# huang-yh/SelfOcc

Measured on NVIDIA H100. Metric: rendered rays/sec (6-cam 900x1600), higher is better.
Workload: dtype f32

## Files before the change

### include/selfocc_b200.h

```cpp
#ifndef SELFOCC_B200_H
#define SELFOCC_B200_H

#include <stdint.h>

#ifdef __cplusplus
extern "C" {
#endif

#define SO_OK 0
#define SO_ERR_INVALID_ARG (-1)
#define SO_ERR_UNSUPPORTED (-2)
#define SO_ERR_CUDA (-3)
#define SO_ERR_NO_DEVICE (-4)

#define SO_ABI_VERSION 9

int so_abi_version(void);
int so_last_cuda_error(void);
const char* so_error_string(int code);
int64_t so_launch_count(void);

#define SO_PROF_NUM_TAGS 10
int so_profile_enable(int on);
int so_profile_reset(void);
// ... 107 lines not shown
                          int32_t n_sem, const uint8_t* lut, uint8_t* occ, uint8_t* sem, void* stream);
int so_occ_sample_labels(const float* vol_sdf, const float* vol_feat, const so_volume_desc* vol_host, const float* xs,
                         int32_t nx, const float* ys, int32_t ny, const float* zs, int32_t nz, const float* points, int64_t m,
                         float thresh, int32_t sem_begin, int32_t n_sem, const uint8_t* lut, uint8_t* occ, uint8_t* sem,
                         void* stream);
int so_occ_confusion(const uint8_t* pred, const uint8_t* gt, const uint8_t* mask, int64_t n, int32_t n_cls, int32_t ignore,
                     int64_t* counts, void* stream);

int so_msda_forward(const float* value, const int64_t* spatial_shapes, const int64_t* level_start_index,
                    const float* loc, const float* weights, float* out,
                    int32_t B, int32_t Nv, int32_t Hd, int32_t Dh, int32_t Nq, int32_t L, int32_t P,
                    void* stream);

int so_msda_backward(const float* value, const int64_t* spatial_shapes, const int64_t* level_start_index,
                     const float* loc, const float* weights, const float* grad_out,
                     float* grad_value, float* grad_loc, float* grad_weights,
                     int32_t B, int32_t Nv, int32_t Hd, int32_t Dh, int32_t Nq, int32_t L, int32_t P,
                     void* stream);

int so_linear_force_ss(int on);
int so_split_tf32(const float* w, float* w_hi, float* w_lo, int64_t n, void* stream);
int so_linear_3xtf32(const float* x, const float* w_hi, const float* w_lo, const float* bias, const float* residual,
                     float* y, int64_t M, int32_t N, int32_t K, int32_t relu, void* stream);

int so_linear_3xtf32_ln(const float* x, const float* w_hi, const float* w_lo, const float* bias, const float* residual,
                        const float* gamma, const float* beta, float eps, float* y, int64_t M, int32_t N, int32_t K,
                        int32_t relu, void* stream);

int so_layer_norm(const float* x, const float* add, const float* gamma, const float* beta, float* y, int64_t rows,
                  int32_t C, float eps, void* stream);

int so_flatten_level(const float* feat, const float* cams_embeds, const float* level_embed, float* out, int32_t N, int32_t C,
                     int32_t hw, int64_t level_start, int64_t total, void* stream);

int so_point_sampling(const float* ref_3d, const float* lidar2img, int32_t D, int32_t Q, int32_t N,
                      float img_h, float img_w, float* uv, uint8_t* mask, uint8_t* vis, void* stream);

int so_point_sampling_scaled(const float* ref_3d, const float* lidar2img, const float* scale_xy, int32_t D,
                             int32_t Q, int32_t N, float img_h, float img_w, float* uv, uint8_t* mask,
                             uint8_t* vis, void* stream);

int so_tpv_cross_attn_forward(const float* value, const int64_t* spatial_shapes,
                              const int64_t* level_start_index, const float* offsets, const float* logits,
                              const float* uv, const uint8_t* vis, float* slots, int32_t* count,
                              int32_t N, int32_t Nv, int32_t Hd, int32_t Dh, int32_t Q, int32_t L, int32_t D,
                              void* stream);

int so_tpv_cross_attn_forward_strided(const float* value, const int64_t* spatial_shapes, const int64_t* level_start_index,
                                      const float* offsets, const float* logits, const float* uv, const uint8_t* vis,
                                      float* slots, int32_t* count, int32_t N, int32_t Nv, int32_t Hd, int32_t Dh, int32_t Q,
                                      int32_t L, int32_t D, int32_t value_ld, int32_t offsets_ld, int32_t logits_ld, void* stream);

int so_attn_force_v1(int on);

int so_visible_index_lists(const uint8_t* mask, int32_t N, int32_t Q, int32_t D,
                           int64_t* index_lists, int32_t* lens, void* stream);

int so_tpv_self_attn_forward(const float* value, const int64_t* spatial_shapes,
                             const int64_t* level_start_index, const float* offsets, const float* logits,
                             const float* ref, float* out,
                             int32_t Nv, int32_t Hd, int32_t Dh, int32_t Q, int32_t L, int32_t P,
                             void* stream);

int so_tpv_self_attn_forward_strided(const float* value, const int64_t* spatial_shapes, const int64_t* level_start_index,
                                     const float* offsets, const float* logits, const float* ref, float* out, int32_t Nv,
                                     int32_t Hd, int32_t Dh, int32_t Q, int32_t L, int32_t P, int32_t value_ld,
                                     int32_t offsets_ld, int32_t logits_ld, void* stream);

int so_tpv_cross_attn_backward(const float* value, const int64_t* spatial_shapes, const int64_t* level_start_index,
                               const float* offsets, const float* logits, const float* uv, const uint8_t* vis,
                               const int32_t* count, const float* grad_slots, float* grad_value, float* grad_offsets,
                               float* grad_logits, int32_t N, int32_t Nv, int32_t Hd, int32_t Dh, int32_t Q, int32_t L,
                               int32_t D, void* stream);

int so_tpv_self_attn_backward(const float* value, const int64_t* spatial_shapes, const int64_t* level_start_index,
                              const float* offsets, const float* logits, const float* ref, const float* grad_out,
                              float* grad_value, float* grad_offsets, float* grad_logits, int32_t Nv, int32_t Hd, int32_t Dh,
                              int32_t Q, int32_t L, int32_t P, void* stream);

#define SO_REPROJ_COMBINE 0
#define SO_REPROJ_MULTI_NEW 1
int so_reproj_stats_forward(const float* weights, const float* ts, const float* deltas, const float* pix,
                            const float* img2prev, const float* img2next, const float* curr_imgs, const float* prev_imgs,
                            const float* next_imgs, int32_t n_cam, int32_t rays_per_cam, int32_t S, int32_t img_h,
                            int32_t img_w, float size_h, float size_w, int32_t mode, float* stats, float* colours,
                            void* stream);
int so_reproj_stats_backward(const float* ts, const float* deltas, const float* pix, const float* img2prev,
                             const float* img2next, const float* curr_imgs, const float* prev_imgs, const float* next_imgs,
                             int32_t n_cam, int32_t rays_per_cam, int32_t S, int32_t img_h, int32_t img_w, float size_h,
                             float size_w, int32_t mode, const float* stats, const float* grad_stats, float* grad_weights,
                             void* stream);

#define SO_SAMPLE_MEAN_EIKONAL 0
#define SO_SAMPLE_MEAN_ABS 1
#define SO_SAMPLE_MEAN_NEG_RELU 2
#define SO_SAMPLE_MEAN_WORKSPACE_BYTES 8192
int so_sample_mean_forward(const float* x, int64_t n, int32_t op, void* workspace, float* out, void* stream);
int so_sample_mean_backward(const float* x, int64_t n, int32_t op, const float* grad_out, float* grad_x, void* stream);

#ifdef __cplusplus
}
#endif
#endif
```

### selfocc_b200/_lib.py

```python
import ctypes as C
import os

_PKG = os.path.dirname(os.path.abspath(__file__))
LIB_PATH = os.environ.get('SELFOCC_B200_LIB') or os.path.join(_PKG, 'lib', 'libselfocc_b200.so')
ABI_VERSION = 9


class AxisMap(C.Structure):
    _fields_ = [('start', C.c_float), ('range0', C.c_float), ('range1', C.c_float), ('size0', C.c_float),
                ('size1', C.c_float), ('offset', C.c_float)]


class VolumeDesc(C.Structure):
    _fields_ = [('H', C.c_int32), ('W', C.c_int32), ('Z', C.c_int32), ('zpitch', C.c_int32),
                ('n_feat', C.c_int32), ('feat_pitch', C.c_int32), ('axis', AxisMap * 3)]


class RayDesc(C.Structure):
    _fields_ = [('n_cam', C.c_int32), ('rays_per_cam', C.c_int32), ('nx', C.c_int32), ('ny', C.c_int32),
                ('sx', C.c_float), ('ox', C.c_float), ('sy', C.c_float), ('oy', C.c_float),
                ('ray_begin', C.c_int64), ('ray_count', C.c_int64), ('chunk_len', C.c_int64)]


class RenderParams(C.Structure):
# ... 6 lines not shown
_I = C.c_int32
_L = C.c_int64
_F = C.c_float

SIGNATURES = {
    'so_abi_version': (C.c_int, []),
    'so_last_cuda_error': (C.c_int, []),
    'so_error_string': (C.c_char_p, [C.c_int]),
    'so_launch_count': (C.c_int64, []),
    'so_profile_enable': (C.c_int, [C.c_int]),
    'so_profile_reset': (C.c_int, []),
    'so_profile_elapsed_ms': (C.c_int, [C.c_int, C.POINTER(C.c_float), C.POINTER(C.c_int32)]),
    'so_tpv_decode': (C.c_int, [_P, _P, _P, _I, _P, _P, _P, _P, C.POINTER(VolumeDesc), _P, _P, _P]),
    'so_tpv_decode_rows': (C.c_int, [_P, _P, _P, _I, _P, _P, _P, _P, C.POINTER(VolumeDesc), _I, _I, _P, _P, _P]),
    'so_tpv_decode_bwd_features': (C.c_int, [_P, _P, _P, _I, C.POINTER(VolumeDesc), _I, _I, _P, _P]),
    'so_tpv_decode_bwd_hidden': (C.c_int, [_P, _P, _P, _P, _I, C.POINTER(VolumeDesc), _I, _I, _P, _P, _P]),
    'so_tpv_decode_bwd_input': (C.c_int, [_P, _P, _L, _P]),
    'so_tpv_decode_force_simt': (C.c_int, [C.c_int]),
    'so_render_train_force_fwd32': (C.c_int, [C.c_int]),
    'so_render_train_force_sem_generic': (C.c_int, [C.c_int]),
    'so_render_workspace_floats': (C.c_int64, [_L]),
    'so_render_infer': (C.c_int, [_P, _P, C.POINTER(VolumeDesc), _P, _P, C.POINTER(RayDesc), C.POINTER(RenderParams),
                                  _P, _P, _P, _P, _P, _P, _P, _P, _P, _P]),
    'so_render_pack_floats': (_L, [C.POINTER(VolumeDesc)]),
    'so_render_pack': (C.c_int, [_P, _P, C.POINTER(VolumeDesc), _P, _P]),
    'so_render_infer_packed': (C.c_int, [_P, _P, C.POINTER(VolumeDesc), _P, _P, _P, C.POINTER(RayDesc), C.POINTER(RenderParams),
                                         _P, _P, _P, _P, _P, _P, _P, _P, _P, _P, _P]),
    'so_render_train_forward': (C.c_int, [_P, _P, C.POINTER(VolumeDesc), _P, _P, C.POINTER(RayDesc), C.POINTER(RenderParams),
                                          _P, _P] + [_P] * 11 + [_P, _P, _P]),
    'so_render_train_pair_floats': (_L, [C.POINTER(VolumeDesc)]),
    'so_render_train_backward': (C.c_int, [_P, _P, C.POINTER(VolumeDesc), _P, _P, C.POINTER(RayDesc), C.POINTER(RenderParams),
                                           _P, _P] + [_P] * 7 + [_P, _P, _P, _P, _P]),
    'so_render_train_probe': (C.c_int, [C.POINTER(VolumeDesc), _P, _P, C.POINTER(RayDesc), C.POINTER(RenderParams), _P, _P, _P]),
    'so_field_query_backward': (C.c_int, [C.POINTER(VolumeDesc), _P, _L, _P, _P, _P, _P, _P, _P]),
    'so_field_second_grad': (C.c_int, [_P, C.POINTER(VolumeDesc), _P, _L, _P, _P]),
    'so_field_second_grad_backward': (C.c_int, [C.POINTER(VolumeDesc), _P, _L, _P, _P, _P]),
    'so_depth_metric_sample': (C.c_int, [_P, _P, _I, _I, _I, _I, _P, _P]),
    'so_depth_metric_sums': (C.c_int, [_P, _P, _P, _P, _I, _I, _P, _P]),
    'so_field_query': (C.c_int, [_P, _P, C.POINTER(VolumeDesc), _P, _L, _P, _P, _P, _P]),
    'so_msda_forward': (C.c_int, [_P, _P, _P, _P, _P, _P, _I, _I, _I, _I, _I, _I, _I, _P]),
    'so_msda_backward': (C.c_int, [_P, _P, _P, _P, _P, _P, _P, _P, _P, _I, _I, _I, _I, _I, _I, _I, _P]),
    'so_linear_force_ss': (C.c_int, [C.c_int]),
    'so_split_tf32': (C.c_int, [_P, _P, _P, _L, _P]),
    'so_linear_3xtf32': (C.c_int, [_P, _P, _P, _P, _P, _P, _L, _I, _I, _I, _P]),
    'so_linear_3xtf32_ln': (C.c_int, [_P, _P, _P, _P, _P, _P, _P, _F, _P, _L, _I, _I, _I, _P]),
    'so_flatten_level': (C.c_int, [_P, _P, _P, _P, _I, _I, _I, _L, _L, _P]),
    'so_layer_norm': (C.c_int, [_P, _P, _P, _P, _P, _L, _I, _F, _P]),
    'so_point_sampling': (C.c_int, [_P, _P, _I, _I, _I, _F, _F, _P, _P, _P, _P]),
    'so_point_sampling_scaled': (C.c_int, [_P, _P, _P, _I, _I, _I, _F, _F, _P, _P, _P, _P]),
    'so_tpv_cross_attn_forward': (C.c_int, [_P, _P, _P, _P, _P, _P, _P, _P, _P, _I, _I, _I, _I, _I, _I, _I, _P]),
    'so_tpv_cross_attn_forward_strided': (C.c_int, [_P, _P, _P, _P, _P, _P, _P, _P, _P] + [_I] * 10 + [_P]),
    'so_tpv_self_attn_forward_strided': (C.c_int, [_P, _P, _P, _P, _P, _P, _P] + [_I] * 9 + [_P]),
    'so_attn_force_v1': (C.c_int, [C.c_int]),
    'so_visible_index_lists': (C.c_int, [_P, _I, _I, _I, _P, _P, _P]),
    'so_tpv_self_attn_forward': (C.c_int, [_P, _P, _P, _P, _P, _P, _P, _I, _I, _I, _I, _I, _I, _P]),
    'so_tpv_cross_attn_backward': (C.c_int, [_P] * 12 + [_I] * 7 + [_P]),
    'so_tpv_self_attn_backward': (C.c_int, [_P] * 10 + [_I] * 6 + [_P]),
    'so_reproj_stats_forward': (C.c_int, [_P] * 9 + [_I] * 5 + [_F, _F, _I, _P, _P, _P]),
    'so_reproj_stats_backward': (C.c_int, [_P] * 8 + [_I] * 5 + [_F, _F, _I, _P, _P, _P, _P]),
    'so_occ_lattice_labels': (C.c_int, [_P, _P, C.POINTER(VolumeDesc), _P, _I, _P, _I, _P, _I, _F, _I, _I, _P, _P, _P, _P]),
    'so_occ_sample_labels': (C.c_int, [_P, _P, C.POINTER(VolumeDesc), _P, _I, _P, _I, _P, _I, _P, _L, _F, _I, _I, _P, _P, _P, _P]),
    'so_occ_confusion': (C.c_int, [_P, _P, _P, _L, _I, _I, _P, _P]),
    'so_sample_mean_forward': (C.c_int, [_P, _L, _I, _P, _P, _P]),
    'so_sample_mean_backward': (C.c_int, [_P, _L, _I, _P, _P, _P]),
}

_lib = None


class SelfOccLibraryError(RuntimeError):
    pass


def load():
    global _lib
    if _lib is not None:
        return _lib
    if not os.path.exists(LIB_PATH):
        raise SelfOccLibraryError(
            'libselfocc_b200.so not found at %s -- run `python -c "import __graft_entry__ as g; g.build()"` '
            '(there is no CPU/PyTorch fallback for the hot path)' % LIB_PATH)
    lib = C.CDLL(LIB_PATH)
    for name, (res, args) in SIGNATURES.items():
        try:
            fn = getattr(lib, name)
        except AttributeError as e:
            raise SelfOccLibraryError('symbol %s missing from %s' % (name, LIB_PATH)) from e
        fn.restype = res
        fn.argtypes = args
    if lib.so_abi_version() != ABI_VERSION:
        raise SelfOccLibraryError('ABI version mismatch: library %d, binding %d' % (lib.so_abi_version(), ABI_VERSION))
    _lib = lib
    return lib


def check(code, what):
    if code != 0:
        lib = load()
        raise SelfOccLibraryError('%s failed: %s (code %d, cudaError %d)' % (
            what, lib.so_error_string(code).decode(), code, lib.so_last_cuda_error()))


def launch_count():
    return int(load().so_launch_count())


# ... 23 lines not shown
```

### selfocc_b200/csrc/gemm.cu

```cuda
#include "tc_common.cuh"

namespace so {

constexpr int kGemmConsumers = 256;
constexpr int kGemmThreads = kGemmConsumers + 32;
constexpr int kGemmTileM = kWgRows;
constexpr int kGemmTileBytes = kGemmTileM * 128;
constexpr int kMaxStages = 12;
constexpr int kMaxBN = 128;

typedef CUresult (*EncodeTiledFn)(CUtensorMap*, CUtensorMapDataType, cuuint32_t, void*, const cuuint64_t*, const cuuint64_t*,
                                  const cuuint32_t*, const cuuint32_t*, CUtensorMapInterleave, CUtensorMapSwizzle,
                                  CUtensorMapL2promotion, CUtensorMapFloatOOBfill);

static EncodeTiledFn get_encode_fn() {
  static EncodeTiledFn fn = nullptr;
  if (!fn) {
    void* p = nullptr;
    cudaDriverEntryPointQueryResult q;
    if (cudaGetDriverEntryPoint("cuTensorMapEncodeTiled", &p, cudaEnableDefault, &q) == cudaSuccess && q == cudaDriverEntryPointSuccess)
      fn = reinterpret_cast<EncodeTiledFn>(p);
  }
  return fn;
}
// ... 38 lines not shown
    const long long c = bn_cost(bn, N, m_tiles, sms, nullptr, nullptr);
    if (c < best_cost) { best = bn; best_cost = c; }
  }
  return best;
}

static PipeCfg make_pipe_cfg(int64_t M, int N, int K, bool reg_a, bool whole_row, int sms) {
  PipeCfg c;
  c.m_tiles = (int)ceil_div64(M, kGemmTileM);
  c.BN = pick_bn(N, c.m_tiles, sms, whole_row);
  bn_cost(c.BN, N, c.m_tiles, sms, &c.n_tiles, &c.groups);
  c.KA = K / kAtomK;
  c.w_bytes = 2 * c.KA * c.BN * 128;
  c.stage_bytes = reg_a ? kGemmTileBytes : 2 * kGemmTileBytes;
  const int fixed = c.w_bytes + 256;
  c.stages = (227 * 1024 - 1024 - fixed) / c.stage_bytes & ~1;
  if (c.stages > kMaxStages) c.stages = kMaxStages;
  c.smem = fixed + c.stages * c.stage_bytes + 1024;
  return c;
}

template <int NR>
__device__ __forceinline__ void fence_regs(float* r) {
#pragma unroll
  for (int i = 0; i < NR; ++i) asm volatile("" : "+f"(r[i])::"memory");
}
template <int NR>
__device__ __forceinline__ void fence_regs(uint32_t* r) {
#pragma unroll
  for (int i = 0; i < NR; ++i) asm volatile("" : "+r"(r[i])::"memory");
}

__device__ __forceinline__ void ring_advance(int& s, uint32_t& ph, int n) {
  if (++s == n) { s = 0; ph ^= 1; }
}

__device__ __forceinline__ void load_split_frag(const uint8_t* stage, int frag_row, int g, int t, uint32_t* ah, uint32_t* al) {
  const uint8_t* r0 = stage + frag_row * 128 + 4 * t;
#pragma unroll
  for (int kk = 0; kk < 4; ++kk) {
    const float v[4] = {*reinterpret_cast<const float*>(r0 + (((2 * kk) ^ g) << 4)),
                        *reinterpret_cast<const float*>(r0 + 8 * 128 + (((2 * kk) ^ g) << 4)),
                        *reinterpret_cast<const float*>(r0 + (((2 * kk + 1) ^ g) << 4)),
                        *reinterpret_cast<const float*>(r0 + 8 * 128 + (((2 * kk + 1) ^ g) << 4))};
#pragma unroll
    for (int i = 0; i < 4; ++i) {
      const float h = tf32_rn(v[i]);
      ah[4 * kk + i] = __float_as_uint(h);
      al[4 * kk + i] = __float_as_uint(v[i] - h);
    }
  }
  fence_regs<16>(ah);
  fence_regs<16>(al);
}

template <int BN>
__device__ __forceinline__ void mma_atom_rs(float* acc, uint32_t* ah, uint32_t* al, uint32_t bhi, uint32_t blo, uint32_t& accum) {
  fence_regs<BN / 2>(acc);
  wg_fence();
#pragma unroll
  for (int prod = 0; prod < 3; ++prod) {
    const uint32_t* af = prod == 1 ? al : ah;
    const uint32_t bb = prod == 2 ? blo : bhi;
#pragma unroll
    for (int kk = 0; kk < kAtomK / 8; ++kk) {
      Wgmma<BN>::rs(acc, af + 4 * kk, make_desc(bb + kk * 32), accum);
      accum = 1u;
    }
  }
  wg_commit();
}

template <int BN, bool kRegA>
__global__ void __launch_bounds__(kGemmThreads, 1)
linear_3xtf32_kernel(const __grid_constant__ CUtensorMap map_x, const __grid_constant__ CUtensorMap map_whi,
                     const __grid_constant__ CUtensorMap map_wlo, const float* __restrict__ bias,
                     const float* __restrict__ residual, float* __restrict__ y, long long M, int N, int KA, int stages,
                     int n_tiles, int m_tiles, int relu, const float* __restrict__ ln_gamma, const float* __restrict__ ln_beta,
                     float ln_eps) {
  constexpr int kStageBytes = kRegA ? kGemmTileBytes : 2 * kGemmTileBytes;
  extern __shared__ uint8_t smem_raw[];
  uint8_t* sm = reinterpret_cast<uint8_t*>((reinterpret_cast<uintptr_t>(smem_raw) + 1023) & ~(uintptr_t)1023);
  const int w_bytes = 2 * KA * BN * 128;
  uint8_t* w_hi = sm;
  uint8_t* w_lo = sm + KA * BN * 128;
  uint8_t* ring = sm + w_bytes;
  uint64_t* bars = reinterpret_cast<uint64_t*>(ring + stages * kStageBytes);
  uint64_t* w_full = bars;
  uint64_t* full = bars + 1;
  uint64_t* empty = full + kMaxStages;
  const int half = stages / 2;

  const int tid = threadIdx.x, warp = tid >> 5, lane = tid & 31;
  const int n_tile = blockIdx.x % n_tiles;
  const int group = blockIdx.x / n_tiles, n_groups = gridDim.x / n_tiles;
  const int n0 = n_tile * BN;

  if (tid == 0) {
    mbar_init(w_full, 1);
    for (int s = 0; s < kMaxStages; ++s) { mbar_init(full + s, 1); mbar_init(empty + s, kGemmConsumers / 2 / 32); }
    asm volatile("fence.mbarrier_init.release.cluster;" ::: "memory");
  }
  __syncthreads();

  if (warp == kGemmConsumers / 32) {
    if (lane == 0) {
      mbar_expect_tx(w_full, (uint32_t)w_bytes);
      for (int a = 0; a < KA; ++a) {
        tma_load_2d(w_hi + a * BN * 128, &map_whi, a * kAtomK, n0, w_full);
        tma_load_2d(w_lo + a * BN * 128, &map_wlo, a * kAtomK, n0, w_full);
      }
      int s0 = 0, s1 = 0; uint32_t ph0 = 0, ph1 = 0;
      constexpr int kPrefetchTiles = 8;
      for (int p = 0; p < kPrefetchTiles; ++p) {
        int mt = group + p * n_groups;
        if (mt < m_tiles)
          for (int a = 0; a < KA; ++a) tma_prefetch_l2_2d(&map_x, a * kAtomK, mt * kGemmTileM);
      }
      int w = 0;
      for (int mt = group; mt < m_tiles; mt += n_groups, w ^= 1) {
        const int mt_pf = mt + kPrefetchTiles * n_groups;
        if (mt_pf < m_tiles)
          for (int a = 0; a < KA; ++a) tma_prefetch_l2_2d(&map_x, a * kAtomK, mt_pf * kGemmTileM);
        for (int a = 0; a < KA; ++a) {
          const int slot = w ? half + s1 : s0;
          mbar_wait(empty + slot, (w ? ph1 : ph0) ^ 1);
          mbar_expect_tx(full + slot, (uint32_t)kGemmTileBytes);
          tma_load_2d(ring + slot * kStageBytes, &map_x, a * kAtomK, mt * kGemmTileM, full + slot);
          if (w) ring_advance(s1, ph1, half); else ring_advance(s0, ph0, half);
        }
      }
    }
    return;
  }

  const int wg = warp >> 2, wl = warp & 3, g = lane >> 2, t = lane & 3;
  const int frag_row = wl * 16 + g;
  float acc[BN / 2];
#pragma unroll
  for (int i = 0; i < BN / 2; ++i) acc[i] = 0.f;
  const uint32_t whi = smem_u32(w_hi), wlo = smem_u32(w_lo);
  mbar_wait(w_full, 0);
  uint8_t* my_ring = ring + wg * half * kStageBytes;
  uint64_t* my_full = full + wg * half;
  uint64_t* my_empty = empty + wg * half;
  int s = 0; uint32_t ph = 0;
  for (int mt = group + wg * n_groups; mt < m_tiles; mt += 2 * n_groups) {
    uint32_t accum = 0;
    if constexpr (kRegA) {
      constexpr bool kTwoSets = BN <= 80;
      uint32_t ah0[16], al0[16], ah1_[kTwoSets ? 16 : 1], al1_[kTwoSets ? 16 : 1];
      uint32_t* ah1 = kTwoSets ? ah1_ : ah0;
      uint32_t* al1 = kTwoSets ? al1_ : al0;
      mbar_wait(my_full + s, ph);
      load_split_frag(my_ring + s * kStageBytes, frag_row, g, t, ah0, al0);
      __syncwarp();
      if (lane == 0) mbar_arrive(my_empty + s);
      ring_advance(s, ph, half);
      for (int a = 0; a < KA; a += 2) {
        mma_atom_rs<BN>(acc, ah0, al0, whi + a * BN * 128, wlo + a * BN * 128, accum);
        if constexpr (kTwoSets) wg_wait1(); else wg_wait0();
        if (a + 1 < KA) {
          mbar_wait(my_full + s, ph);
          load_split_frag(my_ring + s * kStageBytes, frag_row, g, t, ah1, al1);
          __syncwarp();
          if (lane == 0) mbar_arrive(my_empty + s);
          ring_advance(s, ph, half);
          mma_atom_rs<BN>(acc, ah1, al1, whi + (a + 1) * BN * 128, wlo + (a + 1) * BN * 128, accum);
          if constexpr (kTwoSets) wg_wait1(); else wg_wait0();
          if (a + 2 < KA) {
            mbar_wait(my_full + s, ph);
            load_split_frag(my_ring + s * kStageBytes, frag_row, g, t, ah0, al0);
            __syncwarp();
            if (lane == 0) mbar_arrive(my_empty + s);
            ring_advance(s, ph, half);
          }
        }
      }
      wg_wait0();
      fence_regs<BN / 2>(acc);
    } else {
      for (int a = 0; a < KA; ++a) {
        mbar_wait(my_full + s, ph);
        uint8_t* stage = my_ring + s * kStageBytes;
        const uint32_t bhi = whi + a * BN * 128, blo = wlo + a * BN * 128;
        float4* hi = reinterpret_cast<float4*>(stage);
        float4* lo = reinterpret_cast<float4*>(stage + kGemmTileBytes);
        const int wt = tid & 127;
#pragma unroll
        for (int i = 0; i < kGemmTileBytes / 16 / 128; ++i) {
          float4 v = hi[wt + i * 128], h, l;
          h.x = tf32_rn(v.x); l.x = v.x - h.x;
          h.y = tf32_rn(v.y); l.y = v.y - h.y;
          h.z = tf32_rn(v.z); l.z = v.z - h.z;
          h.w = tf32_rn(v.w); l.w = v.w - h.w;
          hi[wt + i * 128] = h;
          lo[wt + i * 128] = l;
        }
        asm volatile("fence.proxy.async.shared::cta;" ::: "memory");
        wg_sync(1 + wg);
        const uint32_t ahi = smem_u32(stage), alo = ahi + kGemmTileBytes;
        fence_regs<BN / 2>(acc);
        wg_fence();
#pragma unroll
        for (int prod = 0; prod < 3; ++prod) {
          const uint32_t ab = prod == 1 ? alo : ahi;
          const uint32_t bb = prod == 2 ? blo : bhi;
#pragma unroll
          for (int kk = 0; kk < kAtomK / 8; ++kk) {
            Wgmma<BN>::ss(acc, make_desc(ab + kk * 32), make_desc(bb + kk * 32), accum);
            accum = 1u;
          }
        }
        wg_commit();
        wg_wait0();
        fence_regs<BN / 2>(acc);
        __syncwarp();
        if (lane == 0) mbar_arrive(my_empty + s);
        ring_advance(s, ph, half);
      }
    }

    const long long row[2] = {(long long)mt * kGemmTileM + frag_row, (long long)mt * kGemmTileM + frag_row + 8};
#pragma unroll
    for (int j = 0; j < BN / 8; ++j) {
      const int gc = n0 + 8 * j + 2 * t;
      const float b0 = (bias && gc < N) ? __ldg(bias + gc) : 0.f, b1 = (bias && gc < N) ? __ldg(bias + gc + 1) : 0.f;
// ... 153 lines not shown
```

### selfocc_b200/csrc/msda.cu

```cuda
#include "common.cuh"
#include <math.h>
#ifndef SO_ATTN_UNROLL
#define SO_ATTN_UNROLL 4
#endif
#ifndef SO_SELF_ATTN_MIN_CTAS
#define SO_SELF_ATTN_MIN_CTAS 4
#endif
#ifndef SO_SELF_ATTN_UNROLL
#define SO_SELF_ATTN_UNROLL 8
#endif
#ifndef SO_ATTN_MIN_CTAS
#define SO_ATTN_MIN_CTAS 5
#endif

namespace so {

constexpr int kMaxLevels = 8;

struct Levels {
  int n;
  int h[kMaxLevels], w[kMaxLevels];
  long long start[kMaxLevels];
};

// ... 210 lines not shown
  if (!live || sg != 0) return;
  float c = (float)max(cnt, 1);
  acc.x /= c; acc.y /= c; acc.z /= c; acc.w /= c;
  *reinterpret_cast<float4*>(slots + item * DH + lc * 4) = acc;
  if (count && h == 0 && lc == 0) count[q] = cnt;
}

template <int DH>
__global__ void __launch_bounds__(256, SO_SELF_ATTN_MIN_CTAS) tpv_self_attn_kernel(const float* __restrict__ value, const long long* __restrict__ shapes, const long long* __restrict__ lsi,
                                                            const float* __restrict__ offsets, const float* __restrict__ logits,
                                                            const float* __restrict__ ref, float* __restrict__ out, int Nv, int Hd,
                                                            int Q, int L, int P, int value_ld, int off_ld, int lg_ld) {
  constexpr int LPI = DH / 4;
  __shared__ Levels lv;
  load_levels(lv, shapes, lsi, L);
  long long t = blockIdx.x * (long long)blockDim.x + threadIdx.x;
  long long item = t / LPI;
  int lc = (int)(t % LPI);
  long long n_items = (long long)Q * Hd;
  bool live = item < n_items;
  if (!live) item = n_items - 1;
  int h = (int)(item % Hd);
  int q = (int)(item / Hd);
  const int pstride = value_ld;
  const int LP = L * P;
  const float* op = offsets + (long long)q * off_ld + (long long)h * LP * 2;
  const float* lg = logits + (long long)q * lg_ld + (long long)h * LP;
  const float* rp = ref + (long long)q * LP * 2;
  float mx, inv_sum;
  softmax_stats<LPI>(lg, LP, lc, mx, inv_sum);
  float4 acc = make_float4(0.f, 0.f, 0.f, 0.f);
  for (int l = 0; l < L; ++l) {
    const int Hl = lv.h[l], Wl = lv.w[l];
    const float rw = 1.0f / (float)Wl, rh = 1.0f / (float)Hl;
    const float* vbase = value + (long long)lv.start[l] * value_ld + h * DH + lc * 4;
    constexpr int kUnroll = SO_SELF_ATTN_UNROLL;
#pragma unroll kUnroll
    for (int p = 0; p < P; ++p) {
      float2 r = __ldg(reinterpret_cast<const float2*>(rp) + l * P + p);
      float2 o = __ldg(reinterpret_cast<const float2*>(op) + l * P + p);
      float aw = __expf(__ldg(lg + l * P + p) - mx) * inv_sum;
      float4 s = bilinear4(vbase, pstride, Hl, Wl, fmaf(o.x, rw, r.x), fmaf(o.y, rh, r.y));
      acc.x = fmaf(aw, s.x, acc.x); acc.y = fmaf(aw, s.y, acc.y);
      acc.z = fmaf(aw, s.z, acc.z); acc.w = fmaf(aw, s.w, acc.w);
    }
  }
  if (live) *reinterpret_cast<float4*>(out + item * DH + lc * 4) = acc;
}

struct SamplePark { float w[4]; int p[4]; };
__device__ __forceinline__ int park_write_slot(int lane) { return (lane & 3) * 8 + (lane >> 2); }
__device__ __forceinline__ int park_read_slot(int lane, int j) { return j * 8 + (lane >> 2); }

__device__ __forceinline__ SamplePark park_sample(float lx, float ly, int Hl, int Wl, int base, float aw) {
  SamplePark s;
  float x = lx * (float)Wl - 0.5f, y = ly * (float)Hl - 0.5f;
  const bool inside = y > -1.f && x > -1.f && y < (float)Hl && x < (float)Wl;
  float xf = floorf(x), yf = floorf(y);
  int x0 = (int)xf, y0 = (int)yf;
  float fx = x - xf, fy = y - yf;
  const bool xa = x0 >= 0, xb = x0 + 1 < Wl, ya = y0 >= 0, yb = y0 + 1 < Hl;
  const float a = inside ? aw : 0.f;
  s.w[0] = (ya && xa) ? a * ((1.f - fy) * (1.f - fx)) : 0.f;
  s.w[1] = (ya && xb) ? a * ((1.f - fy) * fx) : 0.f;
  s.w[2] = (yb && xa) ? a * (fy * (1.f - fx)) : 0.f;
  s.w[3] = (yb && xb) ? a * (fy * fx) : 0.f;
  int xc0 = min(max(x0, 0), Wl - 1), xc1 = min(max(x0 + 1, 0), Wl - 1);
  int yc0 = min(max(y0, 0), Hl - 1), yc1 = min(max(y0 + 1, 0), Hl - 1);
  if (!inside) { xc0 = xc1 = yc0 = yc1 = 0; }
  s.p[0] = base + yc0 * Wl + xc0; s.p[1] = base + yc0 * Wl + xc1;
  s.p[2] = base + yc1 * Wl + xc0; s.p[3] = base + yc1 * Wl + xc1;
  return s;
}

__device__ __forceinline__ void consume_sample(const float4 w, const int4 p, const float* __restrict__ vlane, int value_ld, float4& acc) {
  if (w.x == 0.f && w.y == 0.f && w.z == 0.f && w.w == 0.f) return;
  const float4 v0 = __ldg(reinterpret_cast<const float4*>(vlane + (long long)p.x * value_ld));
  const float4 v1 = __ldg(reinterpret_cast<const float4*>(vlane + (long long)p.y * value_ld));
  const float4 v2 = __ldg(reinterpret_cast<const float4*>(vlane + (long long)p.z * value_ld));
  const float4 v3 = __ldg(reinterpret_cast<const float4*>(vlane + (long long)p.w * value_ld));
  acc.x = fmaf(w.x, v0.x, acc.x); acc.y = fmaf(w.x, v0.y, acc.y); acc.z = fmaf(w.x, v0.z, acc.z); acc.w = fmaf(w.x, v0.w, acc.w);
  acc.x = fmaf(w.y, v1.x, acc.x); acc.y = fmaf(w.y, v1.y, acc.y); acc.z = fmaf(w.y, v1.z, acc.z); acc.w = fmaf(w.y, v1.w, acc.w);
  acc.x = fmaf(w.z, v2.x, acc.x); acc.y = fmaf(w.z, v2.y, acc.y); acc.z = fmaf(w.z, v2.z, acc.z); acc.w = fmaf(w.z, v2.w, acc.w);
  acc.x = fmaf(w.w, v3.x, acc.x); acc.y = fmaf(w.w, v3.y, acc.y); acc.z = fmaf(w.w, v3.z, acc.z); acc.w = fmaf(w.w, v3.w, acc.w);
}

#ifndef SO_ATTN2_MIN_CTAS
#define SO_ATTN2_MIN_CTAS 4
#endif

template <int SPLIT>
__global__ void __launch_bounds__(256, SO_ATTN2_MIN_CTAS) tpv_cross_attn2_kernel(
    const float* __restrict__ value, const long long* __restrict__ shapes, const long long* __restrict__ lsi,
    const float* __restrict__ offsets, const float* __restrict__ logits, const float* __restrict__ uv,
    const unsigned char* __restrict__ vis, float* __restrict__ slots, int* __restrict__ count, int N, int Nv, int Hd, int Q, int L,
    int D, int value_ld, int off_ld, int lg_ld) {
  constexpr int DH = 16, LPI = 4, LANES = LPI * SPLIT;
  __shared__ Levels lv;
  __shared__ float4 park_w[256];
  __shared__ int4 park_p[256];
  load_levels(lv, shapes, lsi, L);
  long long t = blockIdx.x * (long long)blockDim.x + threadIdx.x;
  long long item = t / LANES;
  const int li = (int)(t % LANES);
  const int lc = li % LPI, sg = li / LPI;
  const long long n_items = (long long)Q * Hd;
  const bool live = item < n_items;
  if (!live) item = n_items - 1;
  const int h = (int)(item % Hd);
  const int q = (int)(item / Hd);
  const int LD = L * D;
  const float* op = offsets + (long long)q * off_ld + (long long)h * LD * 2;
  const float* lg = logits + (long long)q * lg_ld + (long long)h * LD;
  float mx, inv_sum;
  softmax_stats<LANES>(lg, LD, li, mx, inv_sum);
  const float* vlane = value + h * DH + lc * 4;
  const int wbase = threadIdx.x & ~31, wl = threadIdx.x & 31;
  const int slot_w = wbase + park_write_slot(wl);
  float4 acc = make_float4(0.f, 0.f, 0.f, 0.f);
  int cnt = 0;
  for (int cam = 0; cam < N; ++cam) {
    const bool visible = __ldg(vis + (long long)cam * Q + q) != 0;
    if (!__any_sync(0xffffffffu, visible)) continue;
    cnt += visible ? 1 : 0;
    const float* uvp = uv + ((long long)cam * Q + q) * D * 2;
    float4 part = make_float4(0.f, 0.f, 0.f, 0.f);
    for (int l = 0; l < L; ++l) {
      const int Hl = lv.h[l], Wl = lv.w[l];
      const float rw = 1.0f / (float)Wl, rh = 1.0f / (float)Hl;
      const int base = cam * Nv + (int)lv.start[l];
      for (int d0 = 0; d0 < D; d0 += LANES) {
        const int d = d0 + li;
        const float2 r = __ldg(reinterpret_cast<const float2*>(uvp) + d);
        const float2 o = __ldg(reinterpret_cast<const float2*>(op) + l * D + d);
        const float aw = visible ? __expf(__ldg(lg + l * D + d) - mx) * inv_sum : 0.f;
        const SamplePark sp = park_sample(fmaf(o.x, rw, r.x), fmaf(o.y, rh, r.y), Hl, Wl, base, aw);
        park_w[slot_w] = make_float4(sp.w[0], sp.w[1], sp.w[2], sp.w[3]);
        park_p[slot_w] = make_int4(sp.p[0], sp.p[1], sp.p[2], sp.p[3]);
        __syncwarp();
#pragma unroll
        for (int j = 0; j < LPI; ++j) {
          const int rs = wbase + park_read_slot(wl, j);
          consume_sample(park_w[rs], park_p[rs], vlane, value_ld, part);
        }
        __syncwarp();
      }
    }
    acc.x += part.x; acc.y += part.y; acc.z += part.z; acc.w += part.w;
  }
#pragma unroll
  for (int s2 = LPI; s2 < LANES; s2 <<= 1) {
    acc.x += __shfl_xor_sync(0xffffffffu, acc.x, s2); acc.y += __shfl_xor_sync(0xffffffffu, acc.y, s2);
    acc.z += __shfl_xor_sync(0xffffffffu, acc.z, s2); acc.w += __shfl_xor_sync(0xffffffffu, acc.w, s2);
  }
  if (!live || sg != 0) return;
  float c = (float)max(cnt, 1);
  acc.x /= c; acc.y /= c; acc.z /= c; acc.w /= c;
  *reinterpret_cast<float4*>(slots + item * DH + lc * 4) = acc;
  if (count && h == 0 && lc == 0) count[q] = cnt;
}

__global__ void __launch_bounds__(256, SO_ATTN2_MIN_CTAS) tpv_self_attn2_kernel(
    const float* __restrict__ value, const long long* __restrict__ shapes, const long long* __restrict__ lsi,
    const float* __restrict__ offsets, const float* __restrict__ logits, const float* __restrict__ ref, float* __restrict__ out, int Nv,
    int Hd, int Q, int L, int P, int value_ld, int off_ld, int lg_ld) {
  constexpr int DH = 16, LPI = 4;
  __shared__ Levels lv;
  __shared__ float4 park_w[256];
  __shared__ int4 park_p[256];
  load_levels(lv, shapes, lsi, L);
  long long t = blockIdx.x * (long long)blockDim.x + threadIdx.x;
  long long item = t / LPI;
  const int lc = (int)(t % LPI);
  const long long n_items = (long long)Q * Hd;
  const bool live = item < n_items;
  if (!live) item = n_items - 1;
  const int h = (int)(item % Hd);
  const int q = (int)(item / Hd);
  const int LP = L * P;
  const float* op = offsets + (long long)q * off_ld + (long long)h * LP * 2;
  const float* lg = logits + (long long)q * lg_ld + (long long)h * LP;
  const float* rp = ref + (long long)q * LP * 2;
  float mx, inv_sum;
  softmax_stats<LPI>(lg, LP, lc, mx, inv_sum);
  const float* vlane = value + h * DH + lc * 4;
  const int wbase = threadIdx.x & ~31, wl = threadIdx.x & 31;
  const int slot_w = wbase + park_write_slot(wl);
  float4 acc = make_float4(0.f, 0.f, 0.f, 0.f);
  for (int l = 0; l < L; ++l) {
    const int Hl = lv.h[l], Wl = lv.w[l];
    const float rw = 1.0f / (float)Wl, rh = 1.0f / (float)Hl;
    const int base = (int)lv.start[l];
    for (int p0 = 0; p0 < P; p0 += LPI) {
      const int p = p0 + lc;
      const float2 r = __ldg(reinterpret_cast<const float2*>(rp) + l * P + p);
      const float2 o = __ldg(reinterpret_cast<const float2*>(op) + l * P + p);
      const float aw = __expf(__ldg(lg + l * P + p) - mx) * inv_sum;
      const SamplePark sp = park_sample(fmaf(o.x, rw, r.x), fmaf(o.y, rh, r.y), Hl, Wl, base, aw);
      park_w[slot_w] = make_float4(sp.w[0], sp.w[1], sp.w[2], sp.w[3]);
// ... 207 lines not shown
  if (vis && ok) vis[cq] = 1;
}

__global__ void zero_bytes_kernel(unsigned char* p, long long n) {
  long long i = blockIdx.x * (long long)blockDim.x + threadIdx.x;
  if (i < n) p[i] = 0;
}

__global__ void __launch_bounds__(1024) visible_index_kernel(const unsigned char* __restrict__ mask, int Q, int D,
                                                             long long* __restrict__ lists, int* __restrict__ lens) {
  __shared__ int warp_cnt[32];
  __shared__ int base;
  int cam = blockIdx.x;
  int lane = threadIdx.x & 31, wid = threadIdx.x >> 5;
  if (threadIdx.x == 0) base = 0;
  __syncthreads();
  for (int q0 = 0; q0 < Q; q0 += 1024) {
    int q = q0 + threadIdx.x;
    bool v = false;
    if (q < Q) {
      const unsigned char* m = mask + ((long long)cam * Q + q) * D;
      for (int d = 0; d < D; ++d) v = v || m[d];
    }
    unsigned bal = __ballot_sync(0xffffffffu, v);
    if (lane == 0) warp_cnt[wid] = __popc(bal);
    __syncthreads();
    int off = base;
    for (int w = 0; w < wid; ++w) off += warp_cnt[w];
    if (v) lists[(long long)cam * Q + off + __popc(bal & ((1u << lane) - 1u))] = q;
    __syncthreads();
    if (threadIdx.x == 0) {
      int tot = 0;
      for (int w = 0; w < 32; ++w) tot += warp_cnt[w];
      base += tot;
    }
    __syncthreads();
  }
  if (threadIdx.x == 0) lens[cam] = base;
}

}

using namespace so;

#define SO_DISPATCH_DH(Dh, EXPR16, EXPR32) \
  do {                                     \
    if ((Dh) == 16) { EXPR16; }            \
    else if ((Dh) == 32) { EXPR32; }       \
    else return SO_ERR_UNSUPPORTED;        \
  } while (0)

static bool g_attn_force_v1 = false;
extern "C" int so_attn_force_v1(int on) { g_attn_force_v1 = on != 0; return SO_OK; }

extern "C" int so_msda_forward(const float* value, const int64_t* spatial_shapes, const int64_t* level_start_index,
                               const float* loc, const float* weights, float* out, int32_t B, int32_t Nv, int32_t Hd,
                               int32_t Dh, int32_t Nq, int32_t L, int32_t P, void* stream) {
  if (!value || !spatial_shapes || !level_start_index || !loc || !weights || !out) return SO_ERR_INVALID_ARG;
  if (B < 1 || Nv < 1 || Hd < 1 || Nq < 0 || L < 1 || P < 1) return SO_ERR_INVALID_ARG;
  if (Nq == 0) return SO_OK;
  cudaStream_t st = (cudaStream_t)stream;
  if (L > kMaxLevels) return SO_ERR_UNSUPPORTED;
  const long long* shp = reinterpret_cast<const long long*>(spatial_shapes);
  const long long* lsi = reinterpret_cast<const long long*>(level_start_index);
  long long threads = (long long)B * Nq * Hd * (Dh / 4);
  unsigned grid = (unsigned)ceil_div64(threads, 256);
  ProfScope prof(4, st);
  SO_DISPATCH_DH(Dh, (msda_forward_kernel<16><<<grid, 256, 0, st>>>(value, shp, lsi, loc, weights, out, B, Nv, Hd, Nq, L, P)),
                 (msda_forward_kernel<32><<<grid, 256, 0, st>>>(value, shp, lsi, loc, weights, out, B, Nv, Hd, Nq, L, P)));
  note_launch(1);
  return check_launch();
}

extern "C" int so_msda_backward(const float* value, const int64_t* spatial_shapes, const int64_t* level_start_index,
                                const float* loc, const float* weights, const float* grad_out, float* grad_value,
                                float* grad_loc, float* grad_weights, int32_t B, int32_t Nv, int32_t Hd, int32_t Dh,
                                int32_t Nq, int32_t L, int32_t P, void* stream) {
  if (!value || !spatial_shapes || !level_start_index || !loc || !weights || !grad_out || !grad_value || !grad_loc ||
      !grad_weights)
    return SO_ERR_INVALID_ARG;
  if (B < 1 || Nv < 1 || Hd < 1 || Nq < 0 || L < 1 || P < 1) return SO_ERR_INVALID_ARG;
  if (Nq == 0) return SO_OK;
  cudaStream_t st = (cudaStream_t)stream;
  if (L > kMaxLevels) return SO_ERR_UNSUPPORTED;
  const long long* shp = reinterpret_cast<const long long*>(spatial_shapes);
  const long long* lsi = reinterpret_cast<const long long*>(level_start_index);
  long long threads = (long long)B * Nq * Hd * (Dh / 4);
  unsigned grid = (unsigned)ceil_div64(threads, 256);
  ProfScope prof(5, st);
  SO_DISPATCH_DH(Dh,
                 (msda_backward_kernel<16><<<grid, 256, 0, st>>>(value, shp, lsi, loc, weights, grad_out, grad_value, grad_loc, grad_weights, B, Nv, Hd, Nq, L, P)),
                 (msda_backward_kernel<32><<<grid, 256, 0, st>>>(value, shp, lsi, loc, weights, grad_out, grad_value, grad_loc, grad_weights, B, Nv, Hd, Nq, L, P)));
  note_launch(1);
  return check_launch();
}

extern "C" int so_point_sampling_scaled(const float* ref_3d, const float* lidar2img, const float* scale_xy, int32_t D,
                                        int32_t Q, int32_t N, float img_h, float img_w, float* uv, uint8_t* mask, uint8_t* vis,
                                        void* stream) {
  if (!ref_3d || !lidar2img || !uv) return SO_ERR_INVALID_ARG;
  if (D < 1 || Q < 1 || N < 1 || !(img_h > 0.f) || !(img_w > 0.f)) return SO_ERR_INVALID_ARG;
  cudaStream_t st = (cudaStream_t)stream;
  if (vis) {
    zero_bytes_kernel<<<(unsigned)ceil_div64((long long)N * Q, 256), 256, 0, st>>>(vis, (long long)N * Q);
    note_launch(1);
  }
  long long n = (long long)N * Q * D;
  point_sampling_kernel<<<(unsigned)ceil_div64(n, 256), 256, 0, st>>>(ref_3d, lidar2img, scale_xy, D, Q, N, img_h, img_w, uv,
                                                                      mask, vis);
  note_launch(1);
  return check_launch();
}

extern "C" int so_point_sampling(const float* ref_3d, const float* lidar2img, int32_t D, int32_t Q, int32_t N, float img_h,
                                 float img_w, float* uv, uint8_t* mask, uint8_t* vis, void* stream) {
  return so_point_sampling_scaled(ref_3d, lidar2img, nullptr, D, Q, N, img_h, img_w, uv, mask, vis, stream);
}

extern "C" int so_tpv_cross_attn_forward_strided(const float* value, const int64_t* spatial_shapes, const int64_t* level_start_index,
                                                 const float* offsets, const float* logits, const float* uv, const uint8_t* vis,
                                                 float* slots, int32_t* count, int32_t N, int32_t Nv, int32_t Hd, int32_t Dh,
                                                 int32_t Q, int32_t L, int32_t D, int32_t value_ld, int32_t offsets_ld,
                                                 int32_t logits_ld, void* stream) {
  if (!value || !spatial_shapes || !level_start_index || !offsets || !logits || !uv || !vis || !slots) return SO_ERR_INVALID_ARG;
  if (N < 1 || Nv < 1 || Hd < 1 || Q < 1 || L < 1 || D < 1) return SO_ERR_INVALID_ARG;
  if (value_ld < Hd * Dh || offsets_ld < Hd * L * D * 2 || logits_ld < Hd * L * D || (value_ld & 3)) return SO_ERR_INVALID_ARG;
  if ((offsets_ld & 1) || (reinterpret_cast<uintptr_t>(offsets) & 7) || (reinterpret_cast<uintptr_t>(value) & 15)) return SO_ERR_INVALID_ARG;
  if (L > kMaxLevels) return SO_ERR_UNSUPPORTED;
  cudaStream_t st = (cudaStream_t)stream;
  const long long* shp = reinterpret_cast<const long long*>(spatial_shapes);
  const long long* lsi = reinterpret_cast<const long long*>(level_start_index);
  const int split = D >= 32 ? 4 : (D >= 16 ? 2 : 1);
  long long threads = (long long)Q * Hd * (Dh / 4) * split;
  unsigned grid = (unsigned)ceil_div64(threads, 256);
  ProfScope prof(2, st);
#define SO_CROSS2(SP) tpv_cross_attn2_kernel<SP><<<grid, 256, 0, st>>>(value, shp, lsi, offsets, logits, uv, vis, slots, count, N, Nv, Hd, Q, L, D, value_ld, offsets_ld, logits_ld)
  if (Dh == 16 && D % (4 * split) == 0 && !g_attn_force_v1 && (long long)N * Nv < (1LL << 31)) {
    if (split == 4) SO_CROSS2(4); else if (split == 2) SO_CROSS2(2); else SO_CROSS2(1);
    note_launch(1);
    return check_launch();
  }
#undef SO_CROSS2
#define SO_CROSS(DHV, SP) tpv_cross_attn_kernel<DHV, SP><<<grid, 256, 0, st>>>(value, shp, lsi, offsets, logits, uv, vis, slots, count, N, Nv, Hd, Q, L, D, value_ld, offsets_ld, logits_ld)
  if (Dh == 16) { if (split == 4) SO_CROSS(16, 4); else if (split == 2) SO_CROSS(16, 2); else SO_CROSS(16, 1); }
  else if (Dh == 32) { if (split == 4) SO_CROSS(32, 4); else if (split == 2) SO_CROSS(32, 2); else SO_CROSS(32, 1); }
  else return SO_ERR_UNSUPPORTED;
#undef SO_CROSS
  note_launch(1);
  return check_launch();
}

extern "C" int so_tpv_cross_attn_forward(const float* value, const int64_t* spatial_shapes, const int64_t* level_start_index,
                                         const float* offsets, const float* logits, const float* uv, const uint8_t* vis,
                                         float* slots, int32_t* count, int32_t N, int32_t Nv, int32_t Hd, int32_t Dh, int32_t Q,
                                         int32_t L, int32_t D, void* stream) {
  return so_tpv_cross_attn_forward_strided(value, spatial_shapes, level_start_index, offsets, logits, uv, vis, slots, count, N, Nv,
                                           Hd, Dh, Q, L, D, Hd * Dh, Hd * L * D * 2, Hd * L * D, stream);
}

extern "C" int so_tpv_self_attn_forward_strided(const float* value, const int64_t* spatial_shapes, const int64_t* level_start_index,
                                                const float* offsets, const float* logits, const float* ref, float* out, int32_t Nv,
                                                int32_t Hd, int32_t Dh, int32_t Q, int32_t L, int32_t P, int32_t value_ld,
                                                int32_t offsets_ld, int32_t logits_ld, void* stream) {
  if (!value || !spatial_shapes || !level_start_index || !offsets || !logits || !ref || !out) return SO_ERR_INVALID_ARG;
  if (Nv < 1 || Hd < 1 || Q < 1 || L < 1 || P < 1) return SO_ERR_INVALID_ARG;
  if (value_ld < Hd * Dh || offsets_ld < Hd * L * P * 2 || logits_ld < Hd * L * P || (value_ld & 3)) return SO_ERR_INVALID_ARG;
  if ((offsets_ld & 1) || (reinterpret_cast<uintptr_t>(offsets) & 7) || (reinterpret_cast<uintptr_t>(value) & 15)) return SO_ERR_INVALID_ARG;
  if (L > kMaxLevels) return SO_ERR_UNSUPPORTED;
  cudaStream_t st = (cudaStream_t)stream;
  const long long* shp = reinterpret_cast<const long long*>(spatial_shapes);
  const long long* lsi = reinterpret_cast<const long long*>(level_start_index);
  long long threads = (long long)Q * Hd * (Dh / 4);
  unsigned grid = (unsigned)ceil_div64(threads, 256);
  ProfScope prof(3, st);
  if (Dh == 16 && P % 4 == 0 && !g_attn_force_v1) {
    tpv_self_attn2_kernel<<<grid, 256, 0, st>>>(value, shp, lsi, offsets, logits, ref, out, Nv, Hd, Q, L, P, value_ld, offsets_ld, logits_ld);
    note_launch(1);
    return check_launch();
  }
  SO_DISPATCH_DH(Dh, (tpv_self_attn_kernel<16><<<grid, 256, 0, st>>>(value, shp, lsi, offsets, logits, ref, out, Nv, Hd, Q, L, P, value_ld, offsets_ld, logits_ld)),
                 (tpv_self_attn_kernel<32><<<grid, 256, 0, st>>>(value, shp, lsi, offsets, logits, ref, out, Nv, Hd, Q, L, P, value_ld, offsets_ld, logits_ld)));
  note_launch(1);
  return check_launch();
}

extern "C" int so_tpv_self_attn_forward(const float* value, const int64_t* spatial_shapes, const int64_t* level_start_index,
                                        const float* offsets, const float* logits, const float* ref, float* out, int32_t Nv,
                                        int32_t Hd, int32_t Dh, int32_t Q, int32_t L, int32_t P, void* stream) {
  return so_tpv_self_attn_forward_strided(value, spatial_shapes, level_start_index, offsets, logits, ref, out, Nv, Hd, Dh, Q, L, P,
                                          Hd * Dh, Hd * L * P * 2, Hd * L * P, stream);
}
// ... 63 lines not shown
```

Measured before the change: 371.0 million.

## Compact visible cross-attention samples into per-warp rings before gathering

Adds a compact variant of the cross-attention kernel. It ballots which sampling points land inside the level and belong to a visible camera, and queues only those into a per-quad shared-memory ring, so that invisible or out-of-bounds samples no longer take gather rounds. It is enabled by default when split==4, with a force flag to select the form. The GEMM also gains an async-proxy fence before releasing ring stages. The ring bookkeeping adds ballots and shared-memory traffic, and the rendered rays metric may not exercise this attention path at all.

```diff
diff --git a/include/selfocc_b200.h b/include/selfocc_b200.h
--- a/include/selfocc_b200.h
+++ b/include/selfocc_b200.h
@@ -183,6 +183,8 @@
                                       int32_t L, int32_t D, int32_t value_ld, int32_t offsets_ld, int32_t logits_ld, void* stream);
 
 int so_attn_force_v1(int on);
+
+int so_cross_attn_force_form(int form);
 
 int so_visible_index_lists(const uint8_t* mask, int32_t N, int32_t Q, int32_t D,
                            int64_t* index_lists, int32_t* lens, void* stream);
diff --git a/selfocc_b200/_lib.py b/selfocc_b200/_lib.py
--- a/selfocc_b200/_lib.py
+++ b/selfocc_b200/_lib.py
@@ -82,6 +82,7 @@
     'so_tpv_cross_attn_forward_strided': (C.c_int, [_P, _P, _P, _P, _P, _P, _P, _P, _P] + [_I] * 10 + [_P]),
     'so_tpv_self_attn_forward_strided': (C.c_int, [_P, _P, _P, _P, _P, _P, _P] + [_I] * 9 + [_P]),
     'so_attn_force_v1': (C.c_int, [C.c_int]),
+    'so_cross_attn_force_form': (C.c_int, [C.c_int]),
     'so_visible_index_lists': (C.c_int, [_P, _I, _I, _I, _P, _P, _P]),
     'so_tpv_self_attn_forward': (C.c_int, [_P, _P, _P, _P, _P, _P, _P, _I, _I, _I, _I, _I, _I, _P]),
     'so_tpv_cross_attn_backward': (C.c_int, [_P] * 12 + [_I] * 7 + [_P]),
diff --git a/selfocc_b200/csrc/gemm.cu b/selfocc_b200/csrc/gemm.cu
--- a/selfocc_b200/csrc/gemm.cu
+++ b/selfocc_b200/csrc/gemm.cu
@@ -114,6 +114,12 @@
   }
   fence_regs<16>(ah);
   fence_regs<16>(al);
+}
+
+__device__ __forceinline__ void release_stage(uint64_t* empty_bar, int lane) {
+  asm volatile("fence.proxy.async.shared::cta;" ::: "memory");
+  __syncwarp();
+  if (lane == 0) mbar_arrive(empty_bar);
 }
 
 template <int BN>
@@ -216,8 +222,7 @@
       uint32_t* al1 = kTwoSets ? al1_ : al0;
       mbar_wait(my_full + s, ph);
       load_split_frag(my_ring + s * kStageBytes, frag_row, g, t, ah0, al0);
-      __syncwarp();
-      if (lane == 0) mbar_arrive(my_empty + s);
+      release_stage(my_empty + s, lane);
       ring_advance(s, ph, half);
       for (int a = 0; a < KA; a += 2) {
         mma_atom_rs<BN>(acc, ah0, al0, whi + a * BN * 128, wlo + a * BN * 128, accum);
@@ -225,16 +230,14 @@
         if (a + 1 < KA) {
           mbar_wait(my_full + s, ph);
           load_split_frag(my_ring + s * kStageBytes, frag_row, g, t, ah1, al1);
-          __syncwarp();
-          if (lane == 0) mbar_arrive(my_empty + s);
+          release_stage(my_empty + s, lane);
           ring_advance(s, ph, half);
           mma_atom_rs<BN>(acc, ah1, al1, whi + (a + 1) * BN * 128, wlo + (a + 1) * BN * 128, accum);
           if constexpr (kTwoSets) wg_wait1(); else wg_wait0();
           if (a + 2 < KA) {
             mbar_wait(my_full + s, ph);
             load_split_frag(my_ring + s * kStageBytes, frag_row, g, t, ah0, al0);
-            __syncwarp();
-            if (lane == 0) mbar_arrive(my_empty + s);
+            release_stage(my_empty + s, lane);
             ring_advance(s, ph, half);
           }
         }
diff --git a/selfocc_b200/csrc/msda.cu b/selfocc_b200/csrc/msda.cu
--- a/selfocc_b200/csrc/msda.cu
+++ b/selfocc_b200/csrc/msda.cu
@@ -286,10 +286,18 @@
 __device__ __forceinline__ int park_write_slot(int lane) { return (lane & 3) * 8 + (lane >> 2); }
 __device__ __forceinline__ int park_read_slot(int lane, int j) { return j * 8 + (lane >> 2); }
 
+__device__ __forceinline__ float2 level_xy(float lx, float ly, int Hl, int Wl) {
+  return make_float2(lx * (float)Wl - 0.5f, ly * (float)Hl - 0.5f);
+}
+__device__ __forceinline__ bool level_inside(float2 p, int Hl, int Wl) {
+  return p.y > -1.f && p.x > -1.f && p.y < (float)Hl && p.x < (float)Wl;
+}
+
 __device__ __forceinline__ SamplePark park_sample(float lx, float ly, int Hl, int Wl, int base, float aw) {
   SamplePark s;
-  float x = lx * (float)Wl - 0.5f, y = ly * (float)Hl - 0.5f;
-  const bool inside = y > -1.f && x > -1.f && y < (float)Hl && x < (float)Wl;
+  const float2 xy = level_xy(lx, ly, Hl, Wl);
+  const float x = xy.x, y = xy.y;
+  const bool inside = level_inside(xy, Hl, Wl);
   float xf = floorf(x), yf = floorf(y);
   int x0 = (int)xf, y0 = (int)yf;
   float fx = x - xf, fy = y - yf;
@@ -323,7 +331,20 @@
 #define SO_ATTN2_MIN_CTAS 4
 #endif
 
-template <int SPLIT>
+__device__ __forceinline__ void park_and_consume(float4* park_w, int4* park_p, int wbase, int wl, int slot_w, float4 w, int4 p,
+                                                 const float* __restrict__ vlane, int value_ld, float4& part) {
+  park_w[slot_w] = w;
+  park_p[slot_w] = p;
+  __syncwarp();
+#pragma unroll
+  for (int j = 0; j < 4; ++j) {
+    const int rs = wbase + park_read_slot(wl, j);
+    consume_sample(park_w[rs], park_p[rs], vlane, value_ld, part);
+  }
+  __syncwarp();
+}
+
+template <int SPLIT, bool COMPACT>
 __global__ void __launch_bounds__(256, SO_ATTN2_MIN_CTAS) tpv_cross_attn2_kernel(
     const float* __restrict__ value, const long long* __restrict__ shapes, const long long* __restrict__ lsi,
     const float* __restrict__ offsets, const float* __restrict__ logits, const float* __restrict__ uv,
@@ -351,6 +372,9 @@
   const float* vlane = value + h * DH + lc * 4;
   const int wbase = threadIdx.x & ~31, wl = threadIdx.x & 31;
   const int slot_w = wbase + park_write_slot(wl);
+  __shared__ float2 ring_xy[COMPACT ? 512 : 1];
+  __shared__ int ring_ld[COMPACT ? 512 : 1];
+  const int ring = 2 * wbase + 8 * (wl >> 2), sj = wl & 3;
   float4 acc = make_float4(0.f, 0.f, 0.f, 0.f);
   int cnt = 0;
   for (int cam = 0; cam < N; ++cam) {
@@ -359,26 +383,62 @@
     cnt += visible ? 1 : 0;
     const float* uvp = uv + ((long long)cam * Q + q) * D * 2;
     float4 part = make_float4(0.f, 0.f, 0.f, 0.f);
-    for (int l = 0; l < L; ++l) {
-      const int Hl = lv.h[l], Wl = lv.w[l];
-      const float rw = 1.0f / (float)Wl, rh = 1.0f / (float)Hl;
-      const int base = cam * Nv + (int)lv.start[l];
-      for (int d0 = 0; d0 < D; d0 += LANES) {
-        const int d = d0 + li;
-        const float2 r = __ldg(reinterpret_cast<const float2*>(uvp) + d);
-        const float2 o = __ldg(reinterpret_cast<const float2*>(op) + l * D + d);
-        const float aw = visible ? __expf(__ldg(lg + l * D + d) - mx) * inv_sum : 0.f;
-        const SamplePark sp = park_sample(fmaf(o.x, rw, r.x), fmaf(o.y, rh, r.y), Hl, Wl, base, aw);
-        park_w[slot_w] = make_float4(sp.w[0], sp.w[1], sp.w[2], sp.w[3]);
-        park_p[slot_w] = make_int4(sp.p[0], sp.p[1], sp.p[2], sp.p[3]);
+    if constexpr (!COMPACT) {
+      for (int l = 0; l < L; ++l) {
+        const int Hl = lv.h[l], Wl = lv.w[l];
+        const float rw = 1.0f / (float)Wl, rh = 1.0f / (float)Hl;
+        const int base = cam * Nv + (int)lv.start[l];
+        for (int d0 = 0; d0 < D; d0 += LANES) {
+          const int d = d0 + li;
+          const float2 r = __ldg(reinterpret_cast<const float2*>(uvp) + d);
+          const float2 o = __ldg(reinterpret_cast<const float2*>(op) + l * D + d);
+          const float aw = visible ? __expf(__ldg(lg + l * D + d) - mx) * inv_sum : 0.f;
+          const SamplePark sp = park_sample(fmaf(o.x, rw, r.x), fmaf(o.y, rh, r.y), Hl, Wl, base, aw);
+          park_and_consume(park_w, park_p, wbase, wl, slot_w, make_float4(sp.w[0], sp.w[1], sp.w[2], sp.w[3]),
+                           make_int4(sp.p[0], sp.p[1], sp.p[2], sp.p[3]), vlane, value_ld, part);
+        }
+      }
+    } else {
+      int head = 0, pending = 0;
+      auto setup_round = [&]() {
         __syncwarp();
-#pragma unroll
-        for (int j = 0; j < LPI; ++j) {
-          const int rs = wbase + park_read_slot(wl, j);
-          consume_sample(park_w[rs], park_p[rs], vlane, value_ld, part);
+        const int take = min(pending, 4);
+        float4 w = make_float4(0.f, 0.f, 0.f, 0.f);
+        int4 p = make_int4(0, 0, 0, 0);
+        if (sj < take) {
+          const int e = ring + ((head + sj) & 7);
+          const float2 xy = ring_xy[e];
+          const int l = ring_ld[e] >> 16, d = ring_ld[e] & 0xffff;
+          const float aw = visible ? __expf(__ldg(lg + l * D + d) - mx) * inv_sum : 0.f;
+          const SamplePark sp = park_sample(xy.x, xy.y, lv.h[l], lv.w[l], cam * Nv + (int)lv.start[l], aw);
+          w = make_float4(sp.w[0], sp.w[1], sp.w[2], sp.w[3]);
+          p = make_int4(sp.p[0], sp.p[1], sp.p[2], sp.p[3]);
         }
-        __syncwarp();
+        park_and_consume(park_w, park_p, wbase, wl, slot_w, w, p, vlane, value_ld, part);
+        head += take;
+        pending -= take;
+      };
+      for (int l = 0; l < L; ++l) {
+        const int Hl = lv.h[l], Wl = lv.w[l];
+        const float rw = 1.0f / (float)Wl, rh = 1.0f / (float)Hl;
+        for (int d0 = 0; d0 < D; d0 += LANES) {
+          const int d = d0 + li;
+          const float2 r = __ldg(reinterpret_cast<const float2*>(uvp) + d);
+          const float2 o = __ldg(reinterpret_cast<const float2*>(op) + l * D + d);
+          const float lx = fmaf(o.x, rw, r.x), ly = fmaf(o.y, rh, r.y);
+          const float2 xy = level_xy(lx, ly, Hl, Wl);
+          const bool keep = level_inside(xy, Hl, Wl) ? visible : !(isfinite(xy.x) && isfinite(xy.y));
+          const unsigned mine = (__ballot_sync(0xffffffffu, keep) >> (wl & ~3)) & 0xfu;
+          if (keep) {
+            const int e = ring + ((head + pending + __popc(mine & ((1u << sj) - 1u))) & 7);
+            ring_xy[e] = make_float2(lx, ly);
+            ring_ld[e] = (l << 16) | d;
+          }
+          pending += __popc(mine);
+          if (__any_sync(0xffffffffu, pending >= 4)) setup_round();
+        }
       }
+      while (__any_sync(0xffffffffu, pending > 0)) setup_round();
     }
     acc.x += part.x; acc.y += part.y; acc.z += part.z; acc.w += part.w;
   }
@@ -692,6 +752,12 @@
 
 static bool g_attn_force_v1 = false;
 extern "C" int so_attn_force_v1(int on) { g_attn_force_v1 = on != 0; return SO_OK; }
+static int g_cross_attn_form = 0;
+extern "C" int so_cross_attn_force_form(int form) {
+  if (form < 0 || form > 2) return SO_ERR_INVALID_ARG;
+  g_cross_attn_form = form;
+  return SO_OK;
+}
 
 extern "C" int so_msda_forward(const float* value, const int64_t* spatial_shapes, const int64_t* level_start_index,
                                const float* loc, const float* weights, float* out, int32_t B, int32_t Nv, int32_t Hd,
@@ -774,9 +840,14 @@
   long long threads = (long long)Q * Hd * (Dh / 4) * split;
   unsigned grid = (unsigned)ceil_div64(threads, 256);
   ProfScope prof(2, st);
-#define SO_CROSS2(SP) tpv_cross_attn2_kernel<SP><<<grid, 256, 0, st>>>(value, shp, lsi, offsets, logits, uv, vis, slots, count, N, Nv, Hd, Q, L, D, value_ld, offsets_ld, logits_ld)
+#define SO_CROSS2(SP, CP) tpv_cross_attn2_kernel<SP, CP><<<grid, 256, 0, st>>>(value, shp, lsi, offsets, logits, uv, vis, slots, count, N, Nv, Hd, Q, L, D, value_ld, offsets_ld, logits_ld)
   if (Dh == 16 && D % (4 * split) == 0 && !g_attn_force_v1 && (long long)N * Nv < (1LL << 31)) {
-    if (split == 4) SO_CROSS2(4); else if (split == 2) SO_CROSS2(2); else SO_CROSS2(1);
+    const bool compact = g_cross_attn_form == 2 || (g_cross_attn_form == 0 && split == 4);
+    if (compact && D < (1 << 16)) {
+      if (split == 4) SO_CROSS2(4, true); else if (split == 2) SO_CROSS2(2, true); else SO_CROSS2(1, true);
+    } else {
+      if (split == 4) SO_CROSS2(4, false); else if (split == 2) SO_CROSS2(2, false); else SO_CROSS2(1, false);
+    }
     note_launch(1);
     return check_launch();
   }
```

After: 372.5 million, median of 6. No clear change (+0.4%).
